# Samsung/tf-fast-rnnt

Hardware: AMD Instinct MI355X
Metric: rnnt_loss_pruned_fwd_bwd_throughput (higher is better)
Workload: dtype f32; 1 GPU; c3: rnnt_loss_pruned fwd+bwd step, B=32/GPU T=1000 S=200 C=500 s_range=5, regular, full boundary, first pass rnnt_loss_simple; global_batch=32, am_pruned=broadcast view

## Files before the change

tf-fast-rnnt_amd/csrc/capi.hip:

```cpp
#include "ftr_common.h"
#ifdef FTR_DIAG
#include "../../include/ftr_diag.h"
#endif
#include <stdlib.h>
#include <string.h>

namespace ftr {
namespace {
thread_local char g_err[512] = {0};
#ifdef FTR_DIAG
int g_mi_impl = -1;
#endif

int device_ok() {
  int n = 0;
  hipError_t e = hipGetDeviceCount(&n);
  if (e != hipSuccess || n <= 0) {
    (void)hipGetLastError();
    set_error("no usable HIP device (%s); this library has no CPU path", e == hipSuccess ? "device count is 0" : hipGetErrorString(e));
    return FTR_ERR_NO_DEVICE;
  }
  return FTR_OK;
}

// ... 635 lines not shown
  FTR_TRY(check_builder(what, B >= 0 && T >= 1 && S >= 0 && C >= 1, termination_symbol, C, true));
  FTR_TRY(check_scale_stride(what, scale_stride));
  if (B == 0) return FTR_OK;
  FTR_TRY(pointers_then_device(what, gpy && prod && lm_probs && am_probs && d_am && (!smoothed || (unigram && am_dot && R)) && (gpx || S == 0) && (symbols || S == 0)));
  return simple_fused_bwd_am(gpx, gpy, Scale{scale, scale_stride, scale_mul}, prod, lm_probs, am_probs, symbols, boundary, termination_symbol, combined_scale, direct_scale, unigram, am_dot, am_only_scale, R, d_am, B, T, S, C, modified, stream_of(stream));
}

int ftr_simple_logprobs_fused_bwd_am_f32(const float* gpx, const float* gpy, const float* scale, int scale_stride,
                                         float scale_mul, const float* prod, const float* lm_probs, const float* am_probs,
                                         const int32_t* symbols, const int32_t* boundary, int termination_symbol,
                                         float* d_am, int B, int T, int S, int C, int modified, void* stream) {
  return fused_bwd_am_entry("simple_logprobs_fused_bwd_am", false, gpx, gpy, scale, scale_stride, scale_mul, prod, lm_probs, am_probs, symbols, boundary, termination_symbol, 1.0f, 1.0f, nullptr, nullptr, 0.0f, nullptr, d_am, B, T, S, C, modified, stream);
}

int ftr_smoothed_logprobs_fused_bwd_am_f32(const float* gpx, const float* gpy, const float* scale, int scale_stride,
                                           float scale_mul, const float* prod, const float* lm_probs,
                                           const float* am_probs, const int32_t* symbols, const int32_t* boundary,
                                           int termination_symbol, float combined_scale, float direct_scale,
                                           const float* unigram, const float* am_dot, float am_only_scale, float* R,
                                           float* d_am, int B, int T, int S, int C, int modified, void* stream) {
  return fused_bwd_am_entry("smoothed_logprobs_fused_bwd_am", true, gpx, gpy, scale, scale_stride, scale_mul, prod, lm_probs, am_probs, symbols, boundary, termination_symbol, combined_scale, direct_scale, unigram, am_dot, am_only_scale, R, d_am, B, T, S, C, modified, stream);
}

int ftr_mutual_information_band_supported(int T, int S, int r) { return mi_band_supported(T, S, r); }

static int pruned_band_fwd_entry(const void* logits, int dtype, const int32_t* symbols, const int32_t* ranges, const int32_t* boundary,
                                 int termination_symbol, double delay_penalty, float* lse, float* px_band, float* py_band,
                                 int B, int T, int S, int C, int r, int modified, int hat, void* stream) {
  const char* what = hat ? "hat_pruned_band_fwd" : "pruned_band_fwd";
  clear_error();
  FTR_TRY(check_builder(what, B >= 0 && T >= 1 && S >= 0 && C >= 1 && r >= 1, termination_symbol, C, false, hat));
  if (B == 0) return FTR_OK;
  FTR_TRY(pointers_then_device(what, logits && ranges && lse && px_band && py_band && (symbols || S == 0)));
  FTR_TRY(lse_rows_dtype(logits, dtype, lse, (size_t)B * T * r, C, termination_symbol, hat, stream_of(stream)));
  return band_gather(logits, dtype, symbols, ranges, boundary, lse, termination_symbol, delay_penalty, px_band, py_band, B, T, S, C, r, modified, hat, stream_of(stream));
}

int ftr_pruned_band_fwd_f32(const float* logits, const int32_t* symbols, const int32_t* ranges, const int32_t* boundary,
                            int termination_symbol, double delay_penalty, float* lse, float* px_band, float* py_band,
                            int B, int T, int S, int C, int r, int modified, void* stream) {
  return pruned_band_fwd_entry(logits, FTR_DTYPE_F32, symbols, ranges, boundary, termination_symbol, delay_penalty, lse, px_band, py_band, B, T, S, C, r, modified, 0, stream);
}

int ftr_hat_pruned_band_fwd_f32(const float* logits, const int32_t* symbols, const int32_t* ranges, const int32_t* boundary,
                                int termination_symbol, double delay_penalty, float* lse, float* px_band, float* py_band,
                                int B, int T, int S, int C, int r, int modified, void* stream) {
// ... 364 lines not shown
```

tf-fast-rnnt_amd/csrc/ftr_common.h:

```cpp
#pragma once
#include <hip/hip_runtime.h>
#include <stdint.h>
#include <stdio.h>
#include <stdarg.h>
#include "../../include/ftr_kd.h"

namespace ftr {

void set_error(const char* fmt, ...);
void clear_error();

inline int check_launch(const char* what) {
  hipError_t e = hipGetLastError();
  if (e != hipSuccess) {
    set_error("%s: launch failed: %s", what, hipGetErrorString(e));
    return FTR_ERR_LAUNCH;
  }
  return FTR_OK;
}

inline int require_rows_32bit(const char* what, size_t rows) {
  if (rows > 0x7fffffffull) {
    set_error("%s: %zu rows (B*T*s_range) exceed the 2^31 - 1 that the launch grids index", what, rows);
    return FTR_ERR_INVALID_ARG;
  }
  return FTR_OK;
}

// ... 151 lines not shown
int prune_ranges(const float* px_grad, const float* py_grad, const int32_t* boundary, int32_t* ranges, int32_t* s_begin, int B, int S, int T, int T1, int r, hipStream_t st);
int do_pruning(const float* am, const float* lm, const int32_t* ranges, float* am_p, float* lm_p, int B, int T, int S1, int C, int r, hipStream_t st);
size_t do_pruning_bwd_workspace_bytes(int B, int T, int S1, int C, int r);
int do_pruning_bwd_ws(const float* g_am_p, const float* g_lm_p, const int32_t* ranges, float* d_am, float* d_lm, int B, int T, int S1, int C, int r, void* ws, size_t ws_bytes, hipStream_t st);
int do_pruning_bwd(const float* g_am_p, const float* g_lm_p, const int32_t* ranges, float* d_am, float* d_lm, int B, int T, int S1, int C, int r, hipStream_t st);
int pruned_logprobs_fwd(const void* logits, int dtype, const int32_t* symbols, const int32_t* ranges, const int32_t* boundary, int blank, double delay_penalty, float* lse, float* px, float* py, int B, int T, int S, int C, int r, int modified, int hat, hipStream_t st);
int pruned_logprobs_bwd(const void* logits, int dtype, const int32_t* symbols, const int32_t* ranges, const int32_t* boundary, int blank, const float* lse, const float* gpx, const float* gpy, Scale scale, void* glogits, int B, int T, int S, int C, int r, int modified, int hat, hipStream_t st);
int simple_rowmax_exp(const float* x, float* probs, float* rowmax, float* rowsum, const float* dotvec, float* dot, size_t rows, int C, hipStream_t st);
int simple_rowmax_exp_pair(const float* x1, float* probs1, float* rowmax1, size_t rows1, const float* x2, float* probs2, float* rowmax2, size_t rows2, int C, hipStream_t st);
int simple_rowdot(const float* x, const float* v, float* dot, size_t rows, int C, hipStream_t st);
size_t simple_colsum_workspace_floats(size_t rows, int C);
int simple_colsum_weighted(const float* x, const float* w, float* out, float* ws, size_t ws_floats, size_t rows, int C, hipStream_t st);
int simple_logprobs_fwd(const float* am, const float* lm, const int32_t* symbols, const float* prod, const float* am_max, const float* lm_max, const int32_t* boundary, int blank, double delay_penalty, const float* lmonly_norm, const float* amonly_norm, const float* ulog, float cs, float ls, float as, float* px, float* py, int B, int T, int S, int C, int modified, hipStream_t st);
int simple_logprobs_bwd_w(const float* gpx, const float* gpy, Scale scale, const float* prod, const int32_t* boundary, float* W, float* rsx, float* rsy, float cs, int B, int T, int S, int modified, hipStream_t st);
int simple_logprobs_bwd_am(const float* gpx, const float* gpy, Scale scale, const float* damp, const float* am_probs, const int32_t* symbols, const int32_t* boundary, int blank, float kdir, const float* uvec, const float* amdot, float as, float* Rout, float* d_am, int B, int T, int S, int C, int modified, hipStream_t st);
int simple_logprobs_bwd_lm(const float* dlmp, const float* lm_probs, const int32_t* symbols, const float* rsx, const float* rsy, int blank, float kdir, const float* arow, const float* invsum, const float* gu, float* d_lm, int B, int S, int C, hipStream_t st);
int simple_fused_supported(int C);
int simple_fused_bwd_supported(int T, int C);
int normalizer_gemm(int kind, const float* x, const float* y, float* out, int B, int T, int S1, int C, hipStream_t st);
int normalizer_gemm_choice(int kind, int B, int T, int S1, int C, int* solution, float* us, float* us_default, int* candidates);
int normalizer_gemm_set_choice(int kind, int B, int T, int S1, int C, int solution);
int simple_fused_fwd(const float* am, const float* lm, const int32_t* symbols, const float* am_probs, const float* lm_probs, const float* am_max, const float* lm_max, const int32_t* boundary, int blank, double delay_penalty, const float* lmonly_norm, const float* amonly_norm, const float* ulog, float cs, float ls, float as, float* px, float* py, float* prod_out, int B, int T, int S, int C, int modified, hipStream_t st);
int simple_fused_bwd_am(const float* gpx, const float* gpy, Scale scale, const float* prod, const float* lm_probs, const float* am_probs, const int32_t* symbols, const int32_t* boundary, int blank, float cs, float kdir, const float* uvec, const float* amdot, float as, float* Rout, float* d_am, int B, int T, int S, int C, int modified, hipStream_t st);
int negated_reduce(const float* ans, int B, int reduction, float* out, hipStream_t st, float sign = -1.0f);
int pruned_kd_fwd(const void* logits, int dtype, const void* teacher, int teacher_dtype, const int32_t* symbols, const int32_t* ranges, const int32_t* boundary, int blank, float temperature, int collapsed, float* node, float* saved, float* utt, int B, int T, int S, int C, int r, hipStream_t st);
int pruned_kd_bwd(const void* logits, int dtype, const void* teacher, int teacher_dtype, const int32_t* symbols, const int32_t* ranges, const int32_t* boundary, int blank, float temperature, int collapsed, const float* saved, Scale scale, void* glogits, int B, int T, int S, int C, int r, hipStream_t st);
int lse_rows(const float* logits, float* lse, size_t rows, int C, int blank, int hat, hipStream_t st);
int lse_rows_dtype(const void* logits, int dtype, float* lse, size_t rows, int C, int blank, int hat, hipStream_t st);
int mi_band_supported(int T, int S, int r);
int band_ranges_check(const int32_t* ranges, const int32_t* boundary, int* flags, int B, int T, int r, hipStream_t st);
int band_gather(const void* logits, int dtype, const int32_t* symbols, const int32_t* ranges, const int32_t* boundary, const float* lse, int blank, double delay_penalty, float* pxb, float* pyb, int B, int T, int S, int C, int r, int modified, int hat, hipStream_t st);
size_t mi_band_workspace_floats(int B, int T, int S, int r);
int mi_band_seg_supported(int T, int S, int r);
size_t mi_band_seg_workspace_floats(int B, int T, int S, int r);
int mi_band_seg(const float* pxb, const float* pyb, const int32_t* ranges, const int32_t* boundary, float* ws, size_t ws_floats, float* ans, float* gxb, float* gyb, int B, int T, int S, int r, int modified, hipStream_t st);
int mi_band(const float* pxb, const float* pyb, const int32_t* ranges, const int32_t* boundary, float* ws, size_t ws_floats, float* ans, float* gxb, float* gyb, int B, int T, int S, int r, int modified, hipStream_t st);
int band_grad_banded(const void* logits, int dtype, const int32_t* symbols, const int32_t* ranges, const int32_t* boundary, int blank, const float* lse, const float* gxb, const float* gyb, Scale scale, void* glogits, int B, int T, int S, int C, int r, int modified, int hat, hipStream_t st);
int selftest(hipStream_t st, int* result_dev);
int debug_stamps(unsigned long long* out16);
int debug_trace(unsigned long long* out, int n);
}
```

tf-fast-rnnt_amd/csrc/simple_fused.hip:

```cpp
#include "ftr_common.h"
#include "launch.h"
#include <cstdlib>

namespace ftr {
namespace {

constexpr float kTinyF = 1.401298464324817e-45f;
template <int MB> struct FusedTile {
  static constexpr int FT = 64 * MB, FK = 32, FLD = FK + 4, NBUF = MB == 1 ? 2 : 1;
};
typedef float v4f __attribute__((ext_vector_type(4)));

constexpr int kGLD = 68;
template <int NS, int MB>
__host__ __device__ constexpr size_t fused_lds_bytes() {
  constexpr size_t tile = FusedTile<MB>::NBUF * (size_t)(FusedTile<MB>::FT + 16 * NS) * FusedTile<MB>::FLD;
  constexpr size_t gather = (size_t)16 * NS * kGLD + 16 * NS + (size_t)16 * NS * 8 + (size_t)FusedTile<MB>::FT * 4;
  return sizeof(float) * (tile > gather ? tile : gather);
}

template <bool MOD, bool SMOOTH, int NS, int MB>
__global__ __launch_bounds__(256, 2) void simple_fused_fwd_kernel(
    const float* __restrict__ am, const float* __restrict__ lm, const int32_t* __restrict__ symbols,
    const float* __restrict__ am_probs, const float* __restrict__ lm_probs, const float* __restrict__ am_max,
// ... 223 lines not shown
      float* yrow = py + ((size_t)b * (S + 1) + s) * T + tq;
      if (tq + 3 < T) *reinterpret_cast<f4u*>(yrow) = vy;
      else { for (int j = 0; j < 4; ++j) if (tq + j < T) yrow[j] = vy[j]; }
      if (prod_out) {
        float* prow = prod_out + ((size_t)b * (S + 1) + s) * T + tq;
        if (tq + 3 < T) *reinterpret_cast<f4u*>(prow) = vp;
        else { for (int j = 0; j < 4; ++j) if (tq + j < T) prow[j] = vp[j]; }
      }
      if (s < S) {
        float* xrow = px + ((size_t)b * S + s) * T1 + tq;
        if (tq + 3 < T1) *reinterpret_cast<f4u*>(xrow) = vx;
        else { for (int j = 0; j < 4; ++j) if (tq + j < T1) xrow[j] = vx[j]; }
      }
    }
  }
}


constexpr int kBT = 64;
constexpr int kBS = 16;
constexpr int kBLT = kBT + 4;
constexpr int kBCB = 16;

__host__ __device__ constexpr size_t fused_bwd_lds_bytes() {
  return sizeof(float) * (2 * kBS * (16 * kBCB) + 2 * kBS * kBLT + 2 * kBS * kBT);
}

template <bool MOD>
__global__ __launch_bounds__(256, 2) void simple_fused_bwd_am_kernel(
    const float* __restrict__ gpx, const float* __restrict__ gpy, const Scale scale, const float* __restrict__ prod,
    const float* __restrict__ lm_probs, const float* __restrict__ am_probs, const int32_t* __restrict__ symbols,
    const int32_t* __restrict__ boundary, int blank, float cs, float kdir, const float* __restrict__ uvec,
    const float* __restrict__ amdot, float as, float* __restrict__ Rout, float* __restrict__ d_am, int T, int S, int C) {
  extern __shared__ __attribute__((aligned(16))) float smem[];
  constexpr int NCB = kBCB, CT = 16 * NCB, LDC = CT, NG = NCB / 4;
  float* lmT = smem;
  float* wT = lmT + 2 * kBS * LDC;
  float* csb = wT + 2 * kBS * kBLT;
  int bx = blockIdx.x, by = blockIdx.y, bz = blockIdx.z;
  {
    const unsigned total = gridDim.x * gridDim.y * gridDim.z;
    if ((total & 7u) == 0) {
      const unsigned lin = blockIdx.x + gridDim.x * (blockIdx.y + gridDim.y * blockIdx.z);
      const unsigned j = (lin & 7u) * (total >> 3) + (lin >> 3);
      by = j % gridDim.y; bx = (j / gridDim.y) % gridDim.x; bz = j / (gridDim.x * gridDim.y);
    }
  }
  const int b = bz, t0 = bx * kBT, c0 = by * CT;
  const int tid = threadIdx.x, lane = tid & 63;
  const int wave = __builtin_amdgcn_readfirstlane(tid >> 6);
  const int T1 = MOD ? T : T + 1;
  const int te = boundary ? boundary[4 * b + 3] : T;
  const float sc = scale.at(b);
  const float* gxb = gpx + (size_t)b * S * T1;
  const float* gyb = gpy + (size_t)b * (S + 1) * T;
  const float* prb = prod + (size_t)b * (S + 1) * T;
  const float* lmb = lm_probs + (size_t)b * (S + 1) * C;
  const int nk = (S + 1 + kBS - 1) / kBS;

  constexpr int NL = (kBS * CT / 4) / 256;
  int lrow[NL], lcol[NL];
  float lmask[NL];
#pragma unroll
  for (int u = 0; u < NL; ++u) {
    const int e = tid + 256 * u, c = c0 + 4 * (e % (CT / 4));
    lrow[u] = e / (CT / 4);
    lcol[u] = min(c, C - 4);
    lmask[u] = c < C ? 1.0f : 0.0f;
  }
  const int wrow = tid >> 4, wq = tid & 15, wt = t0 + 4 * wq;
  const int wtc = min(wt, T - 4);
  const float tmask = wt < T ? 1.0f : 0.0f;
  f4 xmask;
#pragma unroll
  for (int e = 0; e < 4; ++e) xmask[e] = (wt < T && (MOD || wt + e != te)) ? sc : 0.0f;
  struct Stage { f4 lv[NL]; f4 x, y, pr; };
  auto load = [&](int kc, Stage& g, bool want_all) {
    const int s = kc * kBS + wrow;
    const int sy_ = min(s, S), sx_ = min(s, S > 0 ? S - 1 : 0);
    if (want_all) {
#pragma unroll
      for (int u = 0; u < NL; ++u) g.lv[u] = *reinterpret_cast<const f4*>(lmb + (size_t)min(kc * kBS + lrow[u], S) * C + lcol[u]);
      g.y = *reinterpret_cast<const f4u*>(gyb + (size_t)sy_ * T + wtc);
      g.pr = *reinterpret_cast<const f4u*>(prb + (size_t)sy_ * T + wtc);
    }
    g.x = (S > 0) ? (f4)*reinterpret_cast<const f4u*>(gxb + (size_t)sx_ * T1 + wtc) : f4{0.f, 0.f, 0.f, 0.f};
  };
  f4 sx = {0.f, 0.f, 0.f, 0.f}, sy = {0.f, 0.f, 0.f, 0.f};

  v4f acc[NCB];
#pragma unroll
  for (int i = 0; i < NCB; ++i) acc[i] = v4f{0.f, 0.f, 0.f, 0.f};
  const int fk = lane >> 4, fn = lane & 15;

  {
    auto park = [&](int kc, const Stage& g) {
      const int buf = kc & 1;
#pragma unroll
      for (int u = 0; u < NL; ++u) {
        const float m = (kc * kBS + lrow[u] <= S) ? lmask[u] : 0.0f;
        *reinterpret_cast<f4*>(lmT + (buf * kBS + lrow[u]) * LDC + 4 * ((tid + 256 * u) % (CT / 4))) = g.lv[u] * m;
      }
      const int s = kc * kBS + wrow;
      const float rowy = s <= S ? sc * tmask : 0.0f, rowx = s < S ? 1.0f : 0.0f;
      const f4 x = g.x * xmask * rowx, y = g.y * rowy;
      f4 w;
#pragma unroll
      for (int e = 0; e < 4; ++e) w[e] = -cs * (x[e] + y[e]) / (g.pr[e] + kTinyF);
      sx += x; sy += y;
      *reinterpret_cast<f4*>(wT + (buf * kBS + wrow) * kBLT + 4 * wq) = w;
    };
    auto compute = [&](int kc) {
      const int buf = kc & 1;
      const float* abase = lmT + (buf * kBS + fk) * LDC + 4 * fn;
      const float* bbase = wT + (buf * kBS + fk) * kBLT + 16 * wave + fn;
      f4 af[2][NG];
      float bw[kBS / 4];
#pragma unroll
      for (int kk = 0; kk < kBS / 4; ++kk) bw[kk] = bbase[4 * kk * kBLT];
#pragma unroll
      for (int g = 0; g < NG; ++g) af[0][g] = *reinterpret_cast<const f4*>(abase + 64 * g);
#pragma unroll
      for (int kk = 0; kk < kBS / 4; ++kk) {
        if (kk + 1 < kBS / 4) {
#pragma unroll
          for (int g = 0; g < NG; ++g) af[(kk + 1) & 1][g] = *reinterpret_cast<const f4*>(abase + 4 * (kk + 1) * LDC + 64 * g);
        }
        __builtin_amdgcn_sched_barrier(0);
#pragma unroll
        for (int g = 0; g < NG; ++g)
#pragma unroll
          for (int e = 0; e < 4; ++e)
// ... 24 lines not shown
  if (uvec && tok) {
    R = -as * (cx + cy) / amdot[(size_t)b * T + t];
    if (by == 0 && fk == 0) Rout[(size_t)b * T + t] = R;
  }
  const float* aprow = am_probs + ((size_t)b * T + (tok ? t : 0)) * C;
#pragma unroll
  for (int g = 0; g < NG; ++g)
#pragma unroll
    for (int j = 0; j < 4; ++j) {
      const int c = c0 + 64 * g + 16 * fk + 4 * j;
      f4 ap = {0.f, 0.f, 0.f, 0.f};
      if (tok && c < C) ap = *reinterpret_cast<const f4*>(aprow + c);
      if (uvec) {
        f4 uv = {0.f, 0.f, 0.f, 0.f};
        if (c < C) uv = *reinterpret_cast<const f4*>(uvec + c);
#pragma unroll
        for (int e = 0; e < 4; ++e) acc[4 * g + e][j] = ap[e] * (acc[4 * g + e][j] + uv[e] * R);
      } else {
#pragma unroll
        for (int e = 0; e < 4; ++e) acc[4 * g + e][j] = ap[e] * acc[4 * g + e][j];
      }
    }
  {
    constexpr int kB2 = 128;
    static_assert(kB2 * kBT <= 2 * kBS * LDC && kB2 <= 2 * kBS * kBLT, "pass 2 reuses the tiles of pass 1");
    float* xT = lmT;
    int* sym2 = reinterpret_cast<int*>(wT);
    constexpr int kCap = (2 * kBS * kBLT - kB2) * 2;
    unsigned short* rlist = reinterpret_cast<unsigned short*>(wT + kB2);
    int* wcnt = reinterpret_cast<int*>(csb);
    int count = 0;
    const bool listed = S <= 65535;
    __syncthreads();
    if (listed) {
      for (int base = 0; base < S; base += 256) {
        const int srow = base + tid;
        const int sy = srow < S ? min(max(symbols[(size_t)b * S + srow], 0), C - 1) : -1;
        const bool mine = sy >= c0 && sy < c0 + CT;
        const unsigned long long m = __ballot(mine);
        if (lane == 0) wcnt[wave] = __popcll(m);
        __syncthreads();
        int off = count;
        for (int w = 0; w < wave; ++w) off += wcnt[w];
        const int tot = wcnt[0] + wcnt[1] + wcnt[2] + wcnt[3];
        const int at = off + __popcll(m & ((1ull << lane) - 1ull));
        if (mine && at < kCap) rlist[at] = (unsigned short)srow;
        count += tot;
// ... 79 lines not shown
  if (grid.z > 65535) { set_error("simple_logprobs_fused_fwd: B = %d > 65535", B); return FTR_ERR_UNSUPPORTED; }
  const bool smooth = lmonly_norm != nullptr;
  return dispatch(modified != 0, [&](auto mod) {
    return dispatch(smooth, [&](auto sm) {
      return dispatch_among<4, 7, 10, 13>(ns, [&](auto nsv) {
        return dispatch_among<2, 1>(mb, [&](auto mbv) {
          constexpr auto kernel = simple_fused_fwd_kernel<decltype(mod)::value, decltype(sm)::value, decltype(nsv)::value, decltype(mbv)::value>;
          constexpr size_t lds = fused_lds_bytes<decltype(nsv)::value, decltype(mbv)::value>();
          const int rc = reserve_lds<kernel>(lds, "simple_logprobs_fused_fwd");
          if (rc != FTR_OK) return rc;
          hipLaunchKernelGGL(kernel, grid, dim3(256), lds, st, am, lm, symbols, am_probs, lm_probs, am_max, lm_max, boundary, blank,
                             delay_penalty, lmonly_norm, amonly_norm, ulog, cs, ls, as, px, py, prod_out, T, S, C);
          return check_launch("simple_logprobs_fused_fwd");
        });
      });
    });
  });
}

int simple_fused_bwd_supported(int T, int C) {
  return (simple_fused_supported(C) && C >= 4 && T >= 4 && (T % 4) == 0) ? 1 : 0;
}

int simple_fused_bwd_am(const float* gpx, const float* gpy, Scale scale, const float* prod, const float* lm_probs,
                        const float* am_probs, const int32_t* symbols, const int32_t* boundary, int blank, float cs,
                        float kdir, const float* uvec, const float* amdot, float as, float* Rout, float* d_am, int B,
                        int T, int S, int C, int modified, hipStream_t st) {
  if (!simple_fused_bwd_supported(T, C)) {
    set_error("simple_logprobs_fused_bwd_am: T = %d, C = %d is outside the fused kernel's domain (T %% 4 == 0, C %% 4 == 0)", T, C);
    return FTR_ERR_UNSUPPORTED;
  }
  const dim3 grid((T + kBT - 1) / kBT, (C + 16 * kBCB - 1) / (16 * kBCB), B);
  if (grid.z > 65535) { set_error("simple_logprobs_fused_bwd_am: B = %d > 65535", B); return FTR_ERR_UNSUPPORTED; }
  dispatch(modified != 0, [&](auto mod) {
    hipLaunchKernelGGL(simple_fused_bwd_am_kernel<decltype(mod)::value>, grid, dim3(256), fused_bwd_lds_bytes(), st, gpx, gpy, scale, prod, lm_probs, am_probs, symbols, boundary, blank, cs, kdir, uvec, amdot, as, Rout, d_am, T, S, C);
  });
  return check_launch("simple_logprobs_fused_bwd_am");
}

}
```

tf-fast-rnnt_amd/tf_fast_rnnt/_lib.py:

```python
from __future__ import annotations

import ctypes
import os

_HERE = os.path.dirname(os.path.abspath(__file__))
LIB_PATH = os.environ.get("FTR_LIB_PATH") or os.path.join(_HERE, "libftr_hip.so")
_lib = None

_c_fp = ctypes.c_void_p
_c_ip = ctypes.c_void_p
_c_st = ctypes.c_void_p
_c_hi = ctypes.POINTER(ctypes.c_int32)
_i = ctypes.c_int
_f = ctypes.c_float

_SIGNATURES = {
    "ftr_abi_version": (ctypes.c_int, []),
    "ftr_package_version": (ctypes.c_char_p, []),
    "ftr_last_error": (ctypes.c_char_p, []),
    "ftr_mutual_information_workspace_floats": (ctypes.c_size_t, [_i, _i, _i]),
    "ftr_mutual_information_handoff_floats": (ctypes.c_size_t, [_i, _i, _i]),
    "ftr_mutual_information_fwd_f32": (_i, [_c_fp, _c_fp, _c_ip, _c_fp, _c_fp, _i, _i, _i, _i, _c_st]),
    "ftr_mutual_information_bwd_f32": (_i, [_c_fp, _c_fp, _c_ip, _c_fp, _c_fp, _c_fp, _c_fp, _c_fp, _i, _i, _i, _i, _i, _c_st]),
    "ftr_mutual_information_fwd_ws_f32": (_i, [_c_fp, _c_fp, _c_ip, _c_fp, ctypes.c_size_t, _i, _c_fp, _i, _i, _i, _i, _c_st]),
# ... 58 lines not shown
    "ftr_mutual_information_tdt_fwd_f32": (_i, [_c_fp, _c_fp, _c_ip, _c_hi, _i, _c_hi, _i, _c_fp, ctypes.c_size_t, _c_fp, _i, _i, _i, _c_st]),
    "ftr_mutual_information_tdt_bwd_f32": (_i, [_c_fp, _c_fp, _c_ip, _c_hi, _i, _c_hi, _i, _c_fp, ctypes.c_size_t, _c_fp, _c_fp, _c_fp, _i, _i, _i, _c_st]),
    "ftr_mutual_information_viterbi_tdt_workspace_bytes": (ctypes.c_size_t, [_i, _i, _i]),
    "ftr_mutual_information_viterbi_tdt_f32": (_i, [_c_fp, _c_fp, _c_ip, _c_hi, _i, _c_hi, _i, ctypes.c_void_p, ctypes.c_size_t, _c_fp, _c_ip, _c_ip, _c_ip, _i, _i, _i, _c_st]),
    "ftr_tdt_pruned_logprobs_fwd_f32": (_i, [_c_fp, _c_ip, _c_ip, _c_ip, _i, _c_hi, _i, ctypes.c_double, ctypes.c_double, _c_fp, _c_fp, _c_fp, _c_fp, _i, _i, _i, _i, _i, _c_st]),
    "ftr_tdt_pruned_logprobs_bwd_scaled_f32": (_i, [_c_fp, _c_ip, _c_ip, _c_ip, _i, _c_hi, _i, ctypes.c_double, ctypes.c_double, _c_fp, _c_fp, _c_fp, _c_fp, _c_fp, _i, _f, _c_fp, _i, _i, _i, _i, _i, _c_st]),
    "ftr_simple_logprobs_fwd_f32": (_i, [_c_fp, _c_fp, _c_ip, _c_fp, _c_fp, _c_fp, _c_ip, _i, ctypes.c_double, _c_fp, _c_fp, _i, _i, _i, _i, _i, _c_st]),
    "ftr_simple_logprobs_bwd_w_f32": (_i, [_c_fp, _c_fp, _c_fp, _c_ip, _c_fp, _c_fp, _c_fp, _i, _i, _i, _i, _c_st]),
    "ftr_simple_logprobs_bwd_am_f32": (_i, [_c_fp, _c_fp, _c_fp, _c_fp, _c_ip, _c_ip, _i, _c_fp, _i, _i, _i, _i, _i, _c_st]),
    "ftr_simple_logprobs_bwd_lm_f32": (_i, [_c_fp, _c_fp, _c_ip, _c_fp, _c_fp, _i, _c_fp, _i, _i, _i, _c_st]),
    "ftr_selftest": (_i, [ctypes.c_void_p, _c_st]),
}
_LOWP_SIGNATURES = {
    "ftr_pruned_logprobs_fwd_dt": (_i, [_c_fp, _i, _c_ip, _c_ip, _c_ip, _i, ctypes.c_double, _c_fp, _c_fp, _c_fp, _i, _i, _i, _i, _i, _i, _i, _c_st]),
    "ftr_pruned_logprobs_bwd_scaled_dt": (_i, [_c_fp, _i, _c_ip, _c_ip, _c_ip, _i, _c_fp, _c_fp, _c_fp, _c_fp, _i, _f, _c_fp, _i, _i, _i, _i, _i, _i, _i, _c_st]),
    "ftr_pruned_band_fwd_dt": (_i, [_c_fp, _i, _c_ip, _c_ip, _c_ip, _i, ctypes.c_double, _c_fp, _c_fp, _c_fp, _i, _i, _i, _i, _i, _i, _i, _c_st]),
    "ftr_pruned_band_bwd_scaled_dt": (_i, [_c_fp, _i, _c_ip, _c_ip, _c_ip, _i, _c_fp, _c_fp, _c_fp, _c_fp, _i, _f, _c_fp, _i, _i, _i, _i, _i, _i, _i, _c_st]),
}
_KD_SIGNATURES = {
    "ftr_pruned_kd_fwd_dt": (_i, [_c_fp, _i, _c_fp, _i, _c_ip, _c_ip, _c_ip, _i, _f, _i, _c_fp, _c_fp, _c_fp, _i, _i, _i, _i, _i, _c_st]),
    "ftr_pruned_kd_bwd_scaled_dt": (_i, [_c_fp, _i, _c_fp, _i, _c_ip, _c_ip, _c_ip, _i, _f, _i, _c_fp, _c_fp, _i, _f, _c_fp, _i, _i, _i, _i, _i, _c_st]),
    "ftr_pruned_kd_reduce_f32": (_i, [_c_fp, _i, _i, _c_fp, _c_st]),
}
EXPORTED_SYMBOLS = tuple(_SIGNATURES)
LOWP_SYMBOLS = tuple(_LOWP_SIGNATURES)
KD_SYMBOLS = tuple(_KD_SIGNATURES)
FTR_KD_FULL, FTR_KD_COLLAPSED = 0, 1
FTR_MI_WS_CLEAN = 1
FTR_DTYPE_F32, FTR_DTYPE_BF16, FTR_DTYPE_FP16 = 0, 1, 2
FTR_PRUNED_HAT = 1


def lib() -> ctypes.CDLL:
    global _lib
    if _lib is None:
        if not os.path.exists(LIB_PATH):
            raise ImportError(
                f"{LIB_PATH} is missing: build the HIP extension first (python -c 'import __graft_entry__ as g; "
                "g.build()' or make -C tf-fast-rnnt_amd/csrc).  tf_fast_rnnt has no CPU fallback.")
        handle = ctypes.CDLL(LIB_PATH)
        for name, (restype, argtypes) in {**_SIGNATURES, **_LOWP_SIGNATURES, **_KD_SIGNATURES}.items():
            fn = getattr(handle, name)
            fn.restype = restype
            fn.argtypes = argtypes
        _lib = handle
    return _lib


class FtrError(RuntimeError):
    """A native entry point returned an FTR_ERR_* code (the reference raises tf.errors.Internal,
    tf_fast_rnnt_op.cc:114-116)."""


def check(rc: int, what: str) -> None:
    if rc != 1:
        msg = lib().ftr_last_error().decode("utf-8", "replace")
        raise FtrError(f"{what} failed with code {rc}: {msg}")


_profile_hook = None


def set_profile_hook(hook) -> None:
    global _profile_hook
# ... 12 lines not shown
```

tf-fast-rnnt_amd/tf_fast_rnnt/rnnt_loss.py:

```python
from __future__ import annotations

from typing import Optional, Tuple, Union

import ctypes
import os

import torch

from . import _lib
from .mutual_information import (_as_boundary, _ptr, _require_gpu, _stream_ptr, cummin,
                                 mb_forward_backward, mi_forward_backward, mutual_information_recursion,
                                 mutual_information_viterbi, mutual_information_viterbi_tdt, tdt_forward_backward)

_NEG_INF = float("-inf")
_TINY = 1.401298464324817e-45


def tune_normalizer_gemms(enable: bool = True, filename: Optional[str] = None, search: bool = True, when: str = "second") -> None:
    if when not in ("first", "second"):
        raise ValueError("when must be 'first' or 'second'")
    os.environ["FTR_GEMM_TUNE"] = when if (enable and search) else "off"


def normalizer_gemm_choice(kind: int, B: int, T: int, S: int, C: int):
# ... 17 lines not shown


def _check_type(rnnt_type: str) -> None:
    if rnnt_type not in ("regular", "modified", "constrained"):
        raise ValueError(f"rnnt_type should be ('regular' | 'modified' | 'constrained'), given {rnnt_type}")


def _i64(t: torch.Tensor) -> torch.Tensor:
    return t if t.dtype == torch.int64 else t.to(torch.int64)


def fix_for_boundary(px: torch.Tensor, boundary: Optional[torch.Tensor] = None) -> torch.Tensor:
    if boundary is None:
        return px
    B, S, T1 = px.shape
    idx = _i64(boundary[:, 3]).reshape(B, 1, 1).expand(B, S, 1)
    return px.scatter(2, idx, _NEG_INF)


def _use_fused_builder(C: int) -> bool:
    return os.environ.get("FTR_BUILDER_GEMM", "fused") != "library" and bool(_lib.lib().ftr_simple_logprobs_fused_supported(int(C)))


def _use_fused_builder_bwd(T: int, C: int) -> bool:
    mode = os.environ.get("FTR_BUILDER_BWD", "auto")
    if mode == "library" or not _use_fused_builder(C) or not _lib.lib().ftr_simple_logprobs_fused_bwd_supported(int(T), int(C)):
        return False
    return mode == "fused" or C >= 768


def _simple_builder(amc, lmc, symbols, am_probs, lm_probs, am_max, lm_max, boundary, blank, delay_penalty, px, py,
                    B, T, S, C, modified, st):
    if _use_fused_builder(C):
        prod = torch.empty((B, S + 1, T), dtype=torch.float32, device=amc.device)
        _lib.call("ftr_simple_logprobs_fused_fwd_f32", _ptr(amc), _ptr(lmc), _ptr(symbols), _ptr(am_probs), _ptr(lm_probs),
                  _ptr(am_max), _ptr(lm_max), _ptr(boundary), int(blank), float(delay_penalty), _ptr(px), _ptr(py),
                  _ptr(prod), B, T, S, C, int(modified), st)
        return prod
    prod = _gemm(0, lm_probs, am_probs, B, T, S, C, st)
    _lib.call("ftr_simple_logprobs_fwd_f32", _ptr(amc), _ptr(lmc), _ptr(symbols), _ptr(prod), _ptr(am_max),
              _ptr(lm_max), _ptr(boundary), int(blank), float(delay_penalty), _ptr(px), _ptr(py),
              B, T, S, C, int(modified), st)
    return prod


def _simple_forward(lm, am, symbols, termination_symbol, boundary, modified, delay_penalty):
    B, T, C = am.shape
    S = lm.shape[1] - 1
    T1 = T if modified else T + 1
    amc = am.detach().contiguous(); lmc = lm.detach().contiguous()
    dev = amc.device
# ... 7 lines not shown
        _lib.call("ftr_rowmax_exp_pair_f32", _ptr(amc), _ptr(am_probs), _ptr(am_max), B * T,
                  _ptr(lmc), _ptr(lm_probs), _ptr(lm_max), B * (S + 1), C, st)
        prod = _simple_builder(amc, lmc, symbols, am_probs, lm_probs, am_max, lm_max, boundary, termination_symbol,
                               delay_penalty, px, py, B, T, S, C, modified, st)
    return px, py, (am_probs, lm_probs, prod, symbols, boundary), (int(termination_symbol), int(modified))


def _simple_backward(saved, meta, gpx, gpy, scale=None, stride=0, mul=1.0):
    am_probs, lm_probs, prod, symbols, boundary = saved
    blank, modified = meta
    B, T, C = am_probs.shape
    S = lm_probs.shape[1] - 1
    dev = am_probs.device
    gpx = gpx.contiguous(); gpy = gpy.contiguous()
    W = torch.empty_like(prod)
    rsx = torch.empty((B, S + 1), dtype=torch.float32, device=dev)
    rsy = torch.empty((B, S + 1), dtype=torch.float32, device=dev)
    d_am = torch.empty_like(am_probs); d_lm = torch.empty_like(lm_probs)
    with torch.cuda.device(dev):
        st = _stream_ptr(am_probs)
        _lib.call("ftr_simple_logprobs_bwd_w_scaled_f32", _ptr(gpx), _ptr(gpy), _ptr(scale), stride, mul,
                  _ptr(prod), _ptr(boundary), _ptr(W), _ptr(rsx), _ptr(rsy), B, T, S, modified, st)
        dlmp = _gemm(1, W, am_probs, B, T, S, C, st)
        if _use_fused_builder_bwd(T, C):
            _lib.call("ftr_simple_logprobs_fused_bwd_am_f32", _ptr(gpx), _ptr(gpy), _ptr(scale), stride, mul,
                      _ptr(prod), _ptr(lm_probs), _ptr(am_probs), _ptr(symbols), _ptr(boundary), blank, _ptr(d_am),
                      B, T, S, C, modified, st)
        else:
            damp = _gemm(2, W, lm_probs, B, T, S, C, st)
            _lib.call("ftr_simple_logprobs_bwd_am_scaled_f32", _ptr(gpx), _ptr(gpy), _ptr(scale), stride, mul,
                      _ptr(damp), _ptr(am_probs), _ptr(symbols), _ptr(boundary), blank, _ptr(d_am), B, T, S, C,
                      modified, st)
        _lib.call("ftr_simple_logprobs_bwd_lm_f32", _ptr(dlmp), _ptr(lm_probs), _ptr(symbols), _ptr(rsx), _ptr(rsy),
                  blank, _ptr(d_lm), B, S, C, st)
    return d_lm, d_am


class _SimpleLogprobs(torch.autograd.Function):

    @staticmethod
    def forward(ctx, lm, am, symbols, termination_symbol, boundary, modified, delay_penalty):
        px, py, saved, meta = _simple_forward(lm, am, symbols, termination_symbol, boundary, modified, delay_penalty)
        ctx.save_for_backward(*saved)
        ctx.meta = meta
        return px, py

    @staticmethod
    def backward(ctx, gpx, gpy):
        d_lm, d_am = _simple_backward(ctx.saved_tensors, ctx.meta, gpx, gpy)
# ... 1054 lines not shown
                      float(delay_penalty), cs, ls, a_s, _ptr(px), _ptr(py), B, T, S, C, int(modified), st)
    saved = (am_probs, lm_probs, prod, symbols, boundary, inv, u, am_dot)
    meta = (int(termination_symbol), int(modified), cs, ls, a_s, count, process_group)
    return px, py, saved, meta


def _smoothed_backward(saved, meta, gpx, gpy, scale=None, stride=0, mul=1.0):
    am_probs, lm_probs, prod, symbols, boundary, inv, u, am_dot = saved
    blank, modified, cs, ls, a_s, count, group = meta
    B, T, C = am_probs.shape
    S = lm_probs.shape[1] - 1
    dev = am_probs.device
    gpx = gpx.contiguous(); gpy = gpy.contiguous()
    W = torch.empty_like(prod)
    rsx = torch.empty((B, S + 1), dtype=torch.float32, device=dev)
    rsy = torch.empty((B, S + 1), dtype=torch.float32, device=dev)
    R = torch.empty((B, T), dtype=torch.float32, device=dev)
    d_am = torch.empty_like(am_probs); d_lm = torch.empty_like(lm_probs)
    with torch.cuda.device(dev):
        st = _stream_ptr(am_probs)
        _lib.call("ftr_smoothed_logprobs_bwd_w_scaled_f32", _ptr(gpx), _ptr(gpy), _ptr(scale), stride, mul, _ptr(prod),
                  _ptr(boundary), cs, _ptr(W), _ptr(rsx), _ptr(rsy), B, T, S, modified, st)
        dlmp = _gemm(1, W, am_probs, B, T, S, C, st)
        if _use_fused_builder_bwd(T, C):
            _lib.call("ftr_smoothed_logprobs_fused_bwd_am_f32", _ptr(gpx), _ptr(gpy), _ptr(scale), stride, mul, _ptr(prod),
                      _ptr(lm_probs), _ptr(am_probs), _ptr(symbols), _ptr(boundary), blank, cs, cs + a_s, _ptr(u),
                      _ptr(am_dot), a_s, _ptr(R), _ptr(d_am), B, T, S, C, modified, st)
        else:
            damp = _gemm(2, W, lm_probs, B, T, S, C, st)
            _lib.call("ftr_smoothed_logprobs_bwd_am_scaled_f32", _ptr(gpx), _ptr(gpy), _ptr(scale), stride, mul, _ptr(damp),
                      _ptr(am_probs), _ptr(symbols), _ptr(boundary), blank, cs + a_s, _ptr(u), _ptr(am_dot), a_s, _ptr(R),
                      _ptr(d_am), B, T, S, C, modified, st)
        du = _colsum_weighted(am_probs, R, B * T, C, st)
        gul = torch.zeros((C,), dtype=torch.float32, device=dev)
        if S > 0:
            gul.index_add_(0, _i64(symbols).reshape(-1), rsx[:, :S].reshape(-1))
        gul[blank] += rsy.sum()
        du = du + a_s * gul / u
        if group is not None:
            torch.distributed.all_reduce(du, group=group)
        gu = (du / count).contiguous()
        dotq = torch.empty((B, S + 1), dtype=torch.float32, device=dev)
        _lib.call("ftr_rowdot_f32", _ptr(lm_probs), _ptr(gu), _ptr(dotq), B * (S + 1), C, st)
        dotq = dotq * inv
        arow = ((-ls) * (rsx + rsy) - dotq) * inv
        arow = arow.contiguous()
        _lib.call("ftr_smoothed_logprobs_bwd_lm_f32", _ptr(dlmp), _ptr(lm_probs), _ptr(symbols), _ptr(rsx),
                  _ptr(rsy), blank, cs + ls, _ptr(arow), _ptr(inv), _ptr(gu), _ptr(d_lm), B, S, C, st)
    return d_lm, d_am
# ... 103 lines not shown
```

Baseline: 24610 utterances/s.

## Feed precomputed W into fused backward AM kernel and enable it for all C

Adds a variant of the fused backward-AM kernel that reads the already-computed W matrix instead of recomputing it from gpx/gpy/prod, and skips gpx/gpy loads when they are not needed. The fused path is now always used when supported, replacing the separate damp GEMM plus bwd_am kernel for C below 768, which covers this C=500 case. It also templates the column-block count (128 or 256 columns per tile), picking it with a CU-occupancy cost model and raising launch bounds for the narrower tile. The risk is that the fused kernel may be slower than the library GEMM path at small C, and the heuristic may pick a poor tile shape.

Result: faster. 25070 utterances/s (median of 6 runs) (+1.9%).

```diff
diff --git a/include/ftr_fused.h b/include/ftr_fused.h
--- /dev/null
+++ b/include/ftr_fused.h
@@ -0,0 +1,24 @@
+#ifndef FTR_FUSED_H_
+#define FTR_FUSED_H_
+#include "ftr.h"
+
+#ifdef __cplusplus
+extern "C" {
+#endif
+
+int ftr_simple_logprobs_fused_bwd_am_w_f32(const float* gpx, const float* gpy, const float* scale, int scale_stride,
+                                           float scale_mul, const float* W, const float* lm_probs, const float* am_probs,
+                                           const int32_t* symbols, const int32_t* boundary, int termination_symbol,
+                                           float* d_am, int B, int T, int S, int C, int modified, void* stream);
+int ftr_smoothed_logprobs_fused_bwd_am_w_f32(const float* gpx, const float* gpy, const float* scale, int scale_stride,
+                                             float scale_mul, const float* W, const float* lm_probs,
+                                             const float* am_probs, const int32_t* symbols, const int32_t* boundary,
+                                             int termination_symbol, float direct_scale, const float* unigram,
+                                             const float* am_dot, float am_only_scale, float* R, float* d_am, int B, int T,
+                                             int S, int C, int modified, void* stream);
+int ftr_simple_logprobs_fused_bwd_am_w_columns(int B, int T, int C);
+
+#ifdef __cplusplus
+}
+#endif
+#endif
diff --git a/tf-fast-rnnt_amd/csrc/capi.hip b/tf-fast-rnnt_amd/csrc/capi.hip
--- a/tf-fast-rnnt_amd/csrc/capi.hip
+++ b/tf-fast-rnnt_amd/csrc/capi.hip
@@ -681,6 +681,38 @@
   return fused_bwd_am_entry("smoothed_logprobs_fused_bwd_am", true, gpx, gpy, scale, scale_stride, scale_mul, prod, lm_probs, am_probs, symbols, boundary, termination_symbol, combined_scale, direct_scale, unigram, am_dot, am_only_scale, R, d_am, B, T, S, C, modified, stream);
 }
 
+static int fused_bwd_am_w_entry(const char* what, bool smoothed, const float* gpx, const float* gpy, const float* scale,
+                                int scale_stride, float scale_mul, const float* W, const float* lm_probs,
+                                const float* am_probs, const int32_t* symbols, const int32_t* boundary,
+                                int termination_symbol, float direct_scale, const float* unigram, const float* am_dot,
+                                float am_only_scale, float* R, float* d_am, int B, int T, int S, int C, int modified,
+                                void* stream) {
+  clear_error();
+  FTR_TRY(check_builder(what, B >= 0 && T >= 1 && S >= 0 && C >= 1, termination_symbol, C, true));
+  FTR_TRY(check_scale_stride(what, scale_stride));
+  if (B == 0) return FTR_OK;
+  FTR_TRY(pointers_then_device(what, gpy && W && lm_probs && am_probs && d_am && (!smoothed || (unigram && am_dot && R)) && (gpx || S == 0) && (symbols || S == 0)));
+  return simple_fused_bwd_am_w(gpx, gpy, Scale{scale, scale_stride, scale_mul}, W, lm_probs, am_probs, symbols, boundary, termination_symbol, direct_scale, unigram, am_dot, am_only_scale, R, d_am, B, T, S, C, modified, stream_of(stream));
+}
+
+int ftr_simple_logprobs_fused_bwd_am_w_f32(const float* gpx, const float* gpy, const float* scale, int scale_stride,
+                                           float scale_mul, const float* W, const float* lm_probs, const float* am_probs,
+                                           const int32_t* symbols, const int32_t* boundary, int termination_symbol,
+                                           float* d_am, int B, int T, int S, int C, int modified, void* stream) {
+  return fused_bwd_am_w_entry("simple_logprobs_fused_bwd_am_w", false, gpx, gpy, scale, scale_stride, scale_mul, W, lm_probs, am_probs, symbols, boundary, termination_symbol, 1.0f, nullptr, nullptr, 0.0f, nullptr, d_am, B, T, S, C, modified, stream);
+}
+
+int ftr_smoothed_logprobs_fused_bwd_am_w_f32(const float* gpx, const float* gpy, const float* scale, int scale_stride,
+                                             float scale_mul, const float* W, const float* lm_probs,
+                                             const float* am_probs, const int32_t* symbols, const int32_t* boundary,
+                                             int termination_symbol, float direct_scale, const float* unigram,
+                                             const float* am_dot, float am_only_scale, float* R, float* d_am, int B, int T,
+                                             int S, int C, int modified, void* stream) {
+  return fused_bwd_am_w_entry("smoothed_logprobs_fused_bwd_am_w", true, gpx, gpy, scale, scale_stride, scale_mul, W, lm_probs, am_probs, symbols, boundary, termination_symbol, direct_scale, unigram, am_dot, am_only_scale, R, d_am, B, T, S, C, modified, stream);
+}
+
+int ftr_simple_logprobs_fused_bwd_am_w_columns(int B, int T, int C) { return simple_fused_bwd_columns(B, T, C); }
+
 int ftr_mutual_information_band_supported(int T, int S, int r) { return mi_band_supported(T, S, r); }
 
 static int pruned_band_fwd_entry(const void* logits, int dtype, const int32_t* symbols, const int32_t* ranges, const int32_t* boundary,
diff --git a/tf-fast-rnnt_amd/csrc/ftr_common.h b/tf-fast-rnnt_amd/csrc/ftr_common.h
--- a/tf-fast-rnnt_amd/csrc/ftr_common.h
+++ b/tf-fast-rnnt_amd/csrc/ftr_common.h
@@ -4,6 +4,7 @@
 #include <stdio.h>
 #include <stdarg.h>
 #include "../../include/ftr_kd.h"
+#include "../../include/ftr_fused.h"
 
 namespace ftr {
 
@@ -201,6 +202,8 @@
 int normalizer_gemm_set_choice(int kind, int B, int T, int S1, int C, int solution);
 int simple_fused_fwd(const float* am, const float* lm, const int32_t* symbols, const float* am_probs, const float* lm_probs, const float* am_max, const float* lm_max, const int32_t* boundary, int blank, double delay_penalty, const float* lmonly_norm, const float* amonly_norm, const float* ulog, float cs, float ls, float as, float* px, float* py, float* prod_out, int B, int T, int S, int C, int modified, hipStream_t st);
 int simple_fused_bwd_am(const float* gpx, const float* gpy, Scale scale, const float* prod, const float* lm_probs, const float* am_probs, const int32_t* symbols, const int32_t* boundary, int blank, float cs, float kdir, const float* uvec, const float* amdot, float as, float* Rout, float* d_am, int B, int T, int S, int C, int modified, hipStream_t st);
+int simple_fused_bwd_columns(int B, int T, int C);
+int simple_fused_bwd_am_w(const float* gpx, const float* gpy, Scale scale, const float* W, const float* lm_probs, const float* am_probs, const int32_t* symbols, const int32_t* boundary, int blank, float kdir, const float* uvec, const float* amdot, float as, float* Rout, float* d_am, int B, int T, int S, int C, int modified, hipStream_t st);
 int negated_reduce(const float* ans, int B, int reduction, float* out, hipStream_t st, float sign = -1.0f);
 int pruned_kd_fwd(const void* logits, int dtype, const void* teacher, int teacher_dtype, const int32_t* symbols, const int32_t* ranges, const int32_t* boundary, int blank, float temperature, int collapsed, float* node, float* saved, float* utt, int B, int T, int S, int C, int r, hipStream_t st);
 int pruned_kd_bwd(const void* logits, int dtype, const void* teacher, int teacher_dtype, const int32_t* symbols, const int32_t* ranges, const int32_t* boundary, int blank, float temperature, int collapsed, const float* saved, Scale scale, void* glogits, int B, int T, int S, int C, int r, hipStream_t st);
diff --git a/tf-fast-rnnt_amd/csrc/simple_fused.hip b/tf-fast-rnnt_amd/csrc/simple_fused.hip
--- a/tf-fast-rnnt_amd/csrc/simple_fused.hip
+++ b/tf-fast-rnnt_amd/csrc/simple_fused.hip
@@ -269,18 +269,20 @@
 constexpr int kBLT = kBT + 4;
 constexpr int kBCB = 16;
 
+template <int NCB>
 __host__ __device__ constexpr size_t fused_bwd_lds_bytes() {
-  return sizeof(float) * (2 * kBS * (16 * kBCB) + 2 * kBS * kBLT + 2 * kBS * kBT);
-}
-
-template <bool MOD>
-__global__ __launch_bounds__(256, 2) void simple_fused_bwd_am_kernel(
+  return sizeof(float) * (2 * kBS * (16 * NCB) + 2 * kBS * kBLT + 2 * kBS * kBT);
+}
+
+template <bool MOD, bool USEW, int NCB>
+__global__ __launch_bounds__(256, NCB <= 8 ? 4 : 2) void simple_fused_bwd_am_kernel(
     const float* __restrict__ gpx, const float* __restrict__ gpy, const Scale scale, const float* __restrict__ prod,
     const float* __restrict__ lm_probs, const float* __restrict__ am_probs, const int32_t* __restrict__ symbols,
     const int32_t* __restrict__ boundary, int blank, float cs, float kdir, const float* __restrict__ uvec,
     const float* __restrict__ amdot, float as, float* __restrict__ Rout, float* __restrict__ d_am, int T, int S, int C) {
   extern __shared__ __attribute__((aligned(16))) float smem[];
-  constexpr int NCB = kBCB, CT = 16 * NCB, LDC = CT, NG = NCB / 4;
+  constexpr int CT = 16 * NCB, LDC = CT, NG = NCB / 4;
+  static_assert(NCB % 4 == 0 && NCB >= 8 && NCB <= 16, "column blocks come in interleaved groups of four");
   float* lmT = smem;
   float* wT = lmT + 2 * kBS * LDC;
   float* csb = wT + 2 * kBS * kBLT;
@@ -321,6 +323,8 @@
   f4 xmask;
 #pragma unroll
   for (int e = 0; e < 4; ++e) xmask[e] = (wt < T && (MOD || wt + e != te)) ? sc : 0.0f;
+  const bool want_y = !USEW || uvec != nullptr || (blank >= c0 && blank < c0 + CT);
+  const bool want_x = !USEW || uvec != nullptr;
   struct Stage { f4 lv[NL]; f4 x, y, pr; };
   auto load = [&](int kc, Stage& g, bool want_all) {
     const int s = kc * kBS + wrow;
@@ -328,10 +332,10 @@
     if (want_all) {
 #pragma unroll
       for (int u = 0; u < NL; ++u) g.lv[u] = *reinterpret_cast<const f4*>(lmb + (size_t)min(kc * kBS + lrow[u], S) * C + lcol[u]);
-      g.y = *reinterpret_cast<const f4u*>(gyb + (size_t)sy_ * T + wtc);
       g.pr = *reinterpret_cast<const f4u*>(prb + (size_t)sy_ * T + wtc);
-    }
-    g.x = (S > 0) ? (f4)*reinterpret_cast<const f4u*>(gxb + (size_t)sx_ * T1 + wtc) : f4{0.f, 0.f, 0.f, 0.f};
+      if (want_y) g.y = *reinterpret_cast<const f4u*>(gyb + (size_t)sy_ * T + wtc);
+    }
+    if (want_x) g.x = (S > 0) ? (f4)*reinterpret_cast<const f4u*>(gxb + (size_t)sx_ * T1 + wtc) : f4{0.f, 0.f, 0.f, 0.f};
   };
   f4 sx = {0.f, 0.f, 0.f, 0.f}, sy = {0.f, 0.f, 0.f, 0.f};
 
@@ -350,11 +354,17 @@
       }
       const int s = kc * kBS + wrow;
       const float rowy = s <= S ? sc * tmask : 0.0f, rowx = s < S ? 1.0f : 0.0f;
-      const f4 x = g.x * xmask * rowx, y = g.y * rowy;
       f4 w;
-#pragma unroll
-      for (int e = 0; e < 4; ++e) w[e] = -cs * (x[e] + y[e]) / (g.pr[e] + kTinyF);
-      sx += x; sy += y;
+      if (USEW) {
+        w = (s <= S && wt < T) ? g.pr : f4{0.f, 0.f, 0.f, 0.f};
+        if (want_x) sx += g.x * xmask * rowx;
+        if (want_y) sy += g.y * rowy;
+      } else {
+        const f4 x = g.x * xmask * rowx, y = g.y * rowy;
+#pragma unroll
+        for (int e = 0; e < 4; ++e) w[e] = -cs * (x[e] + y[e]) / (g.pr[e] + kTinyF);
+        sx += x; sy += y;
+      }
       *reinterpret_cast<f4*>(wT + (buf * kBS + wrow) * kBLT + 4 * wq) = w;
     };
     auto compute = [&](int kc) {
@@ -425,7 +435,7 @@
       }
     }
   {
-    constexpr int kB2 = 128;
+    constexpr int kB2 = CT / 2;
     static_assert(kB2 * kBT <= 2 * kBS * LDC && kB2 <= 2 * kBS * kBLT, "pass 2 reuses the tiles of pass 1");
     float* xT = lmT;
     int* sym2 = reinterpret_cast<int*>(wT);
@@ -551,20 +561,49 @@
   return (simple_fused_supported(C) && C >= 4 && T >= 4 && (T % 4) == 0) ? 1 : 0;
 }
 
+int simple_fused_bwd_columns(int B, int T, int C) {
+  if (const char* e = getenv("FTR_FUSED_BWD_CT")) { const int v = atoi(e); if (v == 128 || v == 256) return v; }
+  const long long slots_cu = current_device_cus(), ft = (long long)((T + kBT - 1) / kBT) * B;
+  auto cost = [&](int ncb, int wgs) {
+    const long long tiles = ft * ((C + 16 * ncb - 1) / (16 * ncb)), slots = slots_cu * wgs;
+    return ((tiles + slots - 1) / slots) * wgs * ncb;
+  };
+  return cost(8, 4) <= cost(16, 3) ? 128 : 256;
+}
+
+template <bool USEW>
+static int fused_bwd_am_launch(const char* what, int ncb, const float* gpx, const float* gpy, Scale scale, const float* prod_or_w,
+                               const float* lm_probs, const float* am_probs, const int32_t* symbols, const int32_t* boundary,
+                               int blank, float cs, float kdir, const float* uvec, const float* amdot, float as, float* Rout,
+                               float* d_am, int B, int T, int S, int C, int modified, hipStream_t st) {
+  if (!simple_fused_bwd_supported(T, C)) {
+    set_error("%s: T = %d, C = %d is outside the fused kernel's domain (T %% 4 == 0, C %% 4 == 0)", what, T, C);
+    return FTR_ERR_UNSUPPORTED;
+  }
+  const dim3 grid((T + kBT - 1) / kBT, (C + 16 * ncb - 1) / (16 * ncb), B);
+  if (grid.z > 65535) { set_error("%s: B = %d > 65535", what, B); return FTR_ERR_UNSUPPORTED; }
+  dispatch(modified != 0, [&](auto mod) {
+    dispatch_among<8, kBCB>(ncb, [&](auto nb) {
+      constexpr int NCB = USEW ? decltype(nb)::value : kBCB;
+      hipLaunchKernelGGL((simple_fused_bwd_am_kernel<decltype(mod)::value, USEW, NCB>), grid, dim3(256), fused_bwd_lds_bytes<NCB>(), st, gpx, gpy, scale, prod_or_w, lm_probs, am_probs, symbols, boundary, blank, cs, kdir, uvec, amdot, as, Rout, d_am, T, S, C);
+    });
+  });
+  return check_launch(what);
+}
+
 int simple_fused_bwd_am(const float* gpx, const float* gpy, Scale scale, const float* prod, const float* lm_probs,
                         const float* am_probs, const int32_t* symbols, const int32_t* boundary, int blank, float cs,
                         float kdir, const float* uvec, const float* amdot, float as, float* Rout, float* d_am, int B,
                         int T, int S, int C, int modified, hipStream_t st) {
-  if (!simple_fused_bwd_supported(T, C)) {
-    set_error("simple_logprobs_fused_bwd_am: T = %d, C = %d is outside the fused kernel's domain (T %% 4 == 0, C %% 4 == 0)", T, C);
-    return FTR_ERR_UNSUPPORTED;
-  }
-  const dim3 grid((T + kBT - 1) / kBT, (C + 16 * kBCB - 1) / (16 * kBCB), B);
-  if (grid.z > 65535) { set_error("simple_logprobs_fused_bwd_am: B = %d > 65535", B); return FTR_ERR_UNSUPPORTED; }
-  dispatch(modified != 0, [&](auto mod) {
-    hipLaunchKernelGGL(simple_fused_bwd_am_kernel<decltype(mod)::value>, grid, dim3(256), fused_bwd_lds_bytes(), st, gpx, gpy, scale, prod, lm_probs, am_probs, symbols, boundary, blank, cs, kdir, uvec, amdot, as, Rout, d_am, T, S, C);
-  });
-  return check_launch("simple_logprobs_fused_bwd_am");
-}
-
-}
+  return fused_bwd_am_launch<false>("simple_logprobs_fused_bwd_am", kBCB, gpx, gpy, scale, prod, lm_probs, am_probs, symbols, boundary, blank, cs, kdir, uvec, amdot, as, Rout, d_am, B, T, S, C, modified, st);
+}
+
+int simple_fused_bwd_am_w(const float* gpx, const float* gpy, Scale scale, const float* W, const float* lm_probs,
+                          const float* am_probs, const int32_t* symbols, const int32_t* boundary, int blank, float kdir,
+                          const float* uvec, const float* amdot, float as, float* Rout, float* d_am, int B, int T, int S,
+                          int C, int modified, hipStream_t st) {
+  const int ncb = simple_fused_bwd_columns(B, T, C) / 16;
+  return fused_bwd_am_launch<true>("simple_logprobs_fused_bwd_am_w", ncb, gpx, gpy, scale, W, lm_probs, am_probs, symbols, boundary, blank, 1.0f, kdir, uvec, amdot, as, Rout, d_am, B, T, S, C, modified, st);
+}
+
+}
diff --git a/tf-fast-rnnt_amd/tf_fast_rnnt/_lib.py b/tf-fast-rnnt_amd/tf_fast_rnnt/_lib.py
--- a/tf-fast-rnnt_amd/tf_fast_rnnt/_lib.py
+++ b/tf-fast-rnnt_amd/tf_fast_rnnt/_lib.py
@@ -104,9 +104,15 @@
     "ftr_pruned_kd_bwd_scaled_dt": (_i, [_c_fp, _i, _c_fp, _i, _c_ip, _c_ip, _c_ip, _i, _f, _i, _c_fp, _c_fp, _i, _f, _c_fp, _i, _i, _i, _i, _i, _c_st]),
     "ftr_pruned_kd_reduce_f32": (_i, [_c_fp, _i, _i, _c_fp, _c_st]),
 }
+_FUSED_SIGNATURES = {
+    "ftr_simple_logprobs_fused_bwd_am_w_f32": (_i, [_c_fp, _c_fp, _c_fp, _i, _f, _c_fp, _c_fp, _c_fp, _c_ip, _c_ip, _i, _c_fp, _i, _i, _i, _i, _i, _c_st]),
+    "ftr_smoothed_logprobs_fused_bwd_am_w_f32": (_i, [_c_fp, _c_fp, _c_fp, _i, _f, _c_fp, _c_fp, _c_fp, _c_ip, _c_ip, _i, _f, _c_fp, _c_fp, _f, _c_fp, _c_fp, _i, _i, _i, _i, _i, _c_st]),
+    "ftr_simple_logprobs_fused_bwd_am_w_columns": (_i, [_i, _i, _i]),
+}
 EXPORTED_SYMBOLS = tuple(_SIGNATURES)
 LOWP_SYMBOLS = tuple(_LOWP_SIGNATURES)
 KD_SYMBOLS = tuple(_KD_SIGNATURES)
+FUSED_SYMBOLS = tuple(_FUSED_SIGNATURES)
 FTR_KD_FULL, FTR_KD_COLLAPSED = 0, 1
 FTR_MI_WS_CLEAN = 1
 FTR_DTYPE_F32, FTR_DTYPE_BF16, FTR_DTYPE_FP16 = 0, 1, 2
@@ -121,7 +127,7 @@
                 f"{LIB_PATH} is missing: build the HIP extension first (python -c 'import __graft_entry__ as g; "
                 "g.build()' or make -C tf-fast-rnnt_amd/csrc).  tf_fast_rnnt has no CPU fallback.")
         handle = ctypes.CDLL(LIB_PATH)
-        for name, (restype, argtypes) in {**_SIGNATURES, **_LOWP_SIGNATURES, **_KD_SIGNATURES}.items():
+        for name, (restype, argtypes) in {**_SIGNATURES, **_LOWP_SIGNATURES, **_KD_SIGNATURES, **_FUSED_SIGNATURES}.items():
             fn = getattr(handle, name)
             fn.restype = restype
             fn.argtypes = argtypes
diff --git a/tf-fast-rnnt_amd/tf_fast_rnnt/rnnt_loss.py b/tf-fast-rnnt_amd/tf_fast_rnnt/rnnt_loss.py
--- a/tf-fast-rnnt_amd/tf_fast_rnnt/rnnt_loss.py
+++ b/tf-fast-rnnt_amd/tf_fast_rnnt/rnnt_loss.py
@@ -63,11 +63,21 @@
     return os.environ.get("FTR_BUILDER_GEMM", "fused") != "library" and bool(_lib.lib().ftr_simple_logprobs_fused_supported(int(C)))
 
 
-def _use_fused_builder_bwd(T: int, C: int) -> bool:
+_FUSED_BWD_MEASURED = {
+    (32, 512, 100, 500): True,
+    (32, 1000, 200, 500): True,
+    (32, 2000, 300, 1024): True,
+    (8, 8000, 1000, 512): True,
+    (16, 3000, 600, 768): True,
+    (8, 1000, 200, 256): True,
+}
+
+
+def _use_fused_builder_bwd(T: int, C: int, B: int = 1) -> bool:
     mode = os.environ.get("FTR_BUILDER_BWD", "auto")
     if mode == "library" or not _use_fused_builder(C) or not _lib.lib().ftr_simple_logprobs_fused_bwd_supported(int(T), int(C)):
         return False
-    return mode == "fused" or C >= 768
+    return True
 
 
 def _simple_builder(amc, lmc, symbols, am_probs, lm_probs, am_max, lm_max, boundary, blank, delay_penalty, px, py,
@@ -121,9 +131,9 @@
         _lib.call("ftr_simple_logprobs_bwd_w_scaled_f32", _ptr(gpx), _ptr(gpy), _ptr(scale), stride, mul,
                   _ptr(prod), _ptr(boundary), _ptr(W), _ptr(rsx), _ptr(rsy), B, T, S, modified, st)
         dlmp = _gemm(1, W, am_probs, B, T, S, C, st)
-        if _use_fused_builder_bwd(T, C):
-            _lib.call("ftr_simple_logprobs_fused_bwd_am_f32", _ptr(gpx), _ptr(gpy), _ptr(scale), stride, mul,
-                      _ptr(prod), _ptr(lm_probs), _ptr(am_probs), _ptr(symbols), _ptr(boundary), blank, _ptr(d_am),
+        if _use_fused_builder_bwd(T, C, B):
+            _lib.call("ftr_simple_logprobs_fused_bwd_am_w_f32", _ptr(gpx), _ptr(gpy), _ptr(scale), stride, mul,
+                      _ptr(W), _ptr(lm_probs), _ptr(am_probs), _ptr(symbols), _ptr(boundary), blank, _ptr(d_am),
                       B, T, S, C, modified, st)
         else:
             damp = _gemm(2, W, lm_probs, B, T, S, C, st)
@@ -1224,9 +1234,9 @@
         _lib.call("ftr_smoothed_logprobs_bwd_w_scaled_f32", _ptr(gpx), _ptr(gpy), _ptr(scale), stride, mul, _ptr(prod),
                   _ptr(boundary), cs, _ptr(W), _ptr(rsx), _ptr(rsy), B, T, S, modified, st)
         dlmp = _gemm(1, W, am_probs, B, T, S, C, st)
-        if _use_fused_builder_bwd(T, C):
-            _lib.call("ftr_smoothed_logprobs_fused_bwd_am_f32", _ptr(gpx), _ptr(gpy), _ptr(scale), stride, mul, _ptr(prod),
-                      _ptr(lm_probs), _ptr(am_probs), _ptr(symbols), _ptr(boundary), blank, cs, cs + a_s, _ptr(u),
+        if _use_fused_builder_bwd(T, C, B):
+            _lib.call("ftr_smoothed_logprobs_fused_bwd_am_w_f32", _ptr(gpx), _ptr(gpy), _ptr(scale), stride, mul, _ptr(W),
+                      _ptr(lm_probs), _ptr(am_probs), _ptr(symbols), _ptr(boundary), blank, cs + a_s, _ptr(u),
                       _ptr(am_dot), a_s, _ptr(R), _ptr(d_am), B, T, S, C, modified, st)
         else:
             damp = _gemm(2, W, lm_probs, B, T, S, C, st)
```
